# k-dominik/cluster_tools

Hardware: AMD Instinct MI355X
Metric: Gvoxel/s DT-watershed (node, 1/2/4/8 GPU) + % HBM roofline; VI vs ref (higher is better)
Workload: dtype f32

## Files before the change

### cluster_tools_amd/csrc/ctws_api.cpp

```cpp
#include <hip/hip_runtime.h>

#include <algorithm>
#include <chrono>
#include <type_traits>
#include <cmath>
#include <cstdint>
#include <cstdlib>
#include <cstdio>
#include <climits>
#include <cstring>
#include <memory>
#include <string>
#include <thread>
#include <utility>
#include <vector>

#include "../../include/ctws.h"
#include "ctws_kernels.h"
#include "host_pool.h"

using namespace ctws;

namespace {

// ... 11 lines not shown
    uint64_t* W = nullptr;
    uint32_t *Wp = nullptr, *csum = nullptr;
    uint32_t *smin = nullptr, *smax = nullptr, *sb = nullptr, *slmax = nullptr, *soff = nullptr, *surv = nullptr;
    uint32_t *act0 = nullptr, *act1 = nullptr, *lines0 = nullptr, *lines1 = nullptr;
    BlockDesc* desc = nullptr;
    BlockStat* stat = nullptr;
    uint32_t* counter = nullptr;
    double* taps = nullptr;
    int64_t cap_hash = 0;
    uint64_t* hkey = nullptr;
    uint32_t* hpos = nullptr;
    uint32_t* p2err = nullptr;
    int64_t cap_front = 0;
    uint64_t *front0 = nullptr, *front1 = nullptr, *fopen = nullptr;
    uint64_t* fplat = nullptr;
    uint64_t* fseed = nullptr;
    uint32_t* plev = nullptr;
    uint32_t* fflags = nullptr;
    uint32_t *fchunk0 = nullptr, *fchunk1 = nullptr;
    uint32_t *wl0 = nullptr, *wl1 = nullptr, *qgen = nullptr;
    uint32_t* wlcnt = nullptr;
    int64_t cap_fstat = 0;
    uint32_t* fstat = nullptr;
};

constexpr int kCounterBytes = 4 * (4 + 4 * kStatSlots);
constexpr int kFrontierBatch = 8;
constexpr int kFrontierWavesHost = 4;
constexpr int kFrontierMaxIters = 256;
constexpr int kFrontierMaxItersCap = 4096;

}

struct ctws_handle {
    int device = 0;
    hipStream_t stream = nullptr;
    std::string err;
    Workspace ws;
    uint32_t* h_counter = nullptr;
    double* h_taps = nullptr;
    std::vector<std::pair<const char*, float>> timings;
    std::vector<hipEvent_t> events;
    hipEvent_t fev[2] = {nullptr, nullptr};
    uint64_t flood_tiles = 0, flood_iters = 0, flood_lines = 0;
    DevBuf st_in, st_mask, st_init, st_out;
    struct HostSlot {
// ... 17 lines not shown
    DevBuf fs_vals, fs_sorted, fs_off, fs_tmp;
    DevBuf sf_ids, sf_bits, sf_desc, sf_stat, sf_seeds, sf_lab, sf_hm, sf_out;
    DevBuf rg_lab, rg_tab, rg_nodes, rg_pairs, rg_w, rg_keys, rg_skeys, rg_sw, rg_sum, rg_out, rg_tmp, rg_red;
    DevBuf ef_lab, ef_data, ef_nodes, ef_edges, ef_out, ef_ekeys, ef_keys, ef_skeys, ef_tmp, ef_red;
    DevBuf ov_lab, ov_rows;
    DevBuf mo_rows, mo_acc;
    DevBuf rf_data, rf_rows, rf_cnt, rf_off, rf_sums, rf_ctab;
    DevBuf ds_in, ds_out, ds_flag;
    std::vector<uint32_t> ds_flags;
    int64_t sf_n = 0;
    uint64_t sf_lo = 1, sf_hi = 0;
    bool sf_has_bits = false;
    DevBuf tc_P, tc_bits, tc_cnt, tc_offs, tc_woff, tc_red, tc_in, tc_mask, tc_out, tc_raw, tc_tmp, tc_taps;
    DevBuf ev_ka, ev_ca, ev_kb, ev_cb, ev_kp, ev_cp, ev_state, ev_out, ev_stage;
    int64_t ev_cap_a = 0, ev_cap_b = 0, ev_cap_p = 0;
    int stop_after = 0;
    int trace = 0;
    int no_descent = 0;
    int seed_tilecc = 0;
    int no_fallback = 0;
    int force_wide = 0;
    int wide_rerun = 0;
    int sf_sparse = 1;
    int verify = 1;
    int prep_lds = 0;
    int plateau_fill = 1;
    int output_tile = 1;
    int gauss_w = 0;
    int gauss_yx = 1;
    int words_per_wave = 32;
    int d2h_wgs = 0;
    int pack_threads = 6;
    int unpack_threads = 9;
    std::unique_ptr<ctws_host::WorkerPool> pack_pool, unpack_pool;
    int h2d_mode = 0;
    int h2d_wgs = 64;
    int host_ramp = 1;
    int host_batch_blocks = 0;
    int64_t host_batch_voxels = (int64_t)256 << 20;
    int edt_wz = 0;
    int edt_bits = 1;
    int edt_w = 0;
    int fchunk2[3] = {1, 64, 1};
    int fchunk3[3] = {1, 8, 8};
    int fchunk3_masked[3] = {1, 8, 8};
    int fchunk3_env = 0;
// ... 114 lines not shown
        ALLOC(hkey, hash);
        ALLOC(hpos, hash);
        w.cap_hash = hash;
    }
    if (!w.p2err) ALLOC(p2err, 4);
    if (front > w.cap_front) {
        ALLOC(front0, front);
        ALLOC(front1, front);
        ALLOC(fopen, front);
        ALLOC(fplat, front);
        ALLOC(fseed, front);
        ALLOC(fchunk0, (front >> kChunkShift) + 1);
        ALLOC(fchunk1, (front >> kChunkShift) + 1);
        ALLOC(wl0, (front >> kChunkShift) + 1);
        ALLOC(wl1, (front >> kChunkShift) + 1);
        ALLOC(qgen, (front >> kChunkShift) + 1);
        w.cap_front = front;
    }
    if (!w.fflags) ALLOC(fflags, kFrontierBatch);
    if (!w.wlcnt) ALLOC(wlcnt, kFrontierMaxItersCap + 2);
    if (blocks > w.cap_fstat) {
        ALLOC(fstat, 3 * blocks);
        ALLOC(plev, blocks);
        w.cap_fstat = blocks;
    }
    if (!w.counter) ALLOC(counter, kCounterBytes / 4);
    if (!w.taps) ALLOC(taps, 6 * kTapSlot);
#undef ALLOC
    return CTWS_OK;
}

std::vector<double> gaussian_taps(double sigma) {
    std::vector<double> k;
    if (sigma > 0.0) {
        const double sigma2 = -0.5 / sigma / sigma;
        const double norm = 1.0 / (std::sqrt(2.0 * M_PI) * sigma);
        int radius = (int)(3.0 * sigma + 0.5);
        if (radius == 0) radius = 1;
        for (double x = -(double)radius; x <= (double)radius; ++x) {
            const double x2 = x * x;
            k.push_back(norm * std::exp(x2 * sigma2));
        }
    } else {
        k.push_back(1.0);
    }
    double sum = 0.0;
// ... 983 lines not shown
        else
            k_fs_label<uint32_t><<<vg, 256, 0, h->stream>>>(w.desc, w.stat, w.hkey, w.hpos, w.hm, w.lab, w.key, w.cls,
                                                            packed ? 1 : 0);
        k_fs_auto_label<<<vg, 256, 0, h->stream>>>(w.desc, w.stat, w.surv, w.W, w.Wp, w.hm, w.lab, w.key, w.cls,
                                                   packed ? 1 : 0);
    } else {
        if (!cc_seeds)
            k_seed_label<<<rg, 256, 0, h->stream>>>(w.desc, w.stat, w.PF, w.fseed, w.hm, w.lab, w.key, w.cls,
                                                    packed ? 1 : 0);
        k_slice_seed_base<<<gsb, 256, 0, h->stream>>>(w.desc, w.stat, w.W, w.Wp, w.sb);
    }
    LAUNCHCHK();
    mark("seeds");
    if (h->stop_after == CTWS_STOP_SEEDS) {
        HIPCHK(hipStreamSynchronize(h->stream));
        return CTWS_OK;
    }

    int rounds1 = 0, rounds2 = 0;
    h->flood_tiles = h->flood_iters = h->flood_lines = 0;
    float fk1 = 0.f, fk2 = 0.f;
    int fallback = 0, fiters = 0, fiters2 = 0;
    uint32_t* fst = h->trace ? w.fstat : nullptr;
    if (descent) {
        const int dz = pl.nd_ws == 3 ? 16 : 1, dy = pl.nd_ws == 3 ? 16 : 64, dx = pl.nd_ws == 3 ? 16 : 64;
        const dim3 dg(tiles8(((maxZ + dz - 1) / dz) * ((maxY + dy - 1) / dy) * ((maxX + dx - 1) / dx)), nb);
        {
            if (pl.nd_ws == 3) k_descent_tile<3><<<dg, 512, 0, h->stream>>>(w.desc, w.stat, w.hm, w.lab, cc, w.fseed, w.P);
            else k_descent_tile<2><<<dg, 512, 0, h->stream>>>(w.desc, w.stat, w.hm, w.lab, cc, w.fseed, w.P);
            LAUNCHCHK();
        }
        mark("descent_tile");
        if (fst) HIPCHK(hipMemsetAsync(fst, 0, sizeof(uint32_t) * 2 * (size_t)nb, h->stream));
        bool any_mask = false;
        for (int i = 0; i < nb; ++i) any_mask |= desc[i].mask != nullptr;
        const bool plat_fill = h->plateau_fill && packed && any_mask;
        if (plat_fill) HIPCHK(hipMemsetAsync(w.plev, 0, sizeof(uint32_t) * (size_t)nb, h->stream));
        k_descent_init<8><<<wtg, 256, 0, h->stream>>>(w.desc, w.stat, w.hm, w.P, w.key, w.cls, w.fopen,
                                                     w.front0, fst, plat_fill ? w.plev : nullptr);
        LAUNCHCHK();
        if (plat_fill) {
            HIPCHK(hipMemsetAsync(w.fplat, 0, sizeof(uint64_t) * (size_t)TF, h->stream));
            k_plat_mark<<<wtg, 256, 0, h->stream>>>(w.desc, w.stat, w.hm, w.plev, w.fopen, w.fplat);
            LAUNCHCHK();
        }
        mark("flood_descent");
// ... 8 lines not shown
            k_plat_scan_col<1><<<dim3(cols_g, nb), 256, 0, h->stream>>>(w.desc, w.stat, w.key, w.fplat, w.plev);
            if (pl.nd_ws == 3)
                k_plat_scan_col<2><<<dim3(cols_g, nb), 256, 0, h->stream>>>(w.desc, w.stat, w.key, w.fplat, w.plev);
            k_plat_restore<<<dim3((unsigned)std::min<int64_t>(((int64_t)maxZ * maxY * ((maxX + 63) / 64) + 255) / 256, 4096), nb), 256, 0, h->stream>>>(w.desc, w.stat, w.fopen, w.fplat,
                                                                                  w.front0);
            LAUNCHCHK();
            if ((r = run_frontier(h, pl, nb, TF, max_tiles, TT, packed, fst, &fiters, &rounds1, &fk1)) != CTWS_OK)
                return r;
        }
        mark("flood_relax");
        if (fst) {
            std::vector<uint32_t> hs(2 * (size_t)nb);
            HIPCHK(hipMemcpyAsync(hs.data(), fst, sizeof(uint32_t) * 2 * (size_t)nb, hipMemcpyDeviceToHost, h->stream));
            HIPCHK(hipStreamSynchronize(h->stream));
            double no = 0, nv = 0;
            for (int i = 0; i < nb; ++i) {
                no += hs[i];
                nv += hs[nb + i];
            }
            add_timing(h, "open_voxels", (float)no);
            add_timing(h, "frontier_visits", (float)nv);
        }
        HIPCHK(hipMemsetAsync(w.counter, 0, 40, h->stream));
        if (pl.nd_ws == 3)
            k_flood_verify<3><<<wtg, 256, 0, h->stream>>>(w.desc, w.stat, w.hm, w.key, w.fopen, w.counter);
        else
            k_flood_verify<2><<<wtg, 256, 0, h->stream>>>(w.desc, w.stat, w.hm, w.key, w.fopen, w.counter);
        LAUNCHCHK();
        if (h->verify) {
            HIPCHK(hipMemcpyAsync(h->h_counter, w.counter, 40, hipMemcpyDeviceToHost, h->stream));
            HIPCHK(hipStreamSynchronize(h->stream));
            if (h->trace && h->h_counter[0]) {
                fprintf(stderr, "[ctws] flood verify: violations at");
                for (uint32_t k = 0; k < std::min(8u, h->h_counter[1]); ++k) fprintf(stderr, " %u", h->h_counter[2 + k]);
                fprintf(stderr, "\n");
            }
            if (h->h_counter[0] && h->verify >= 2) {
                h->err = "flood fixpoint check failed (CTWS_VERIFY=2)";
                return CTWS_EHIP;
            }
            if (h->h_counter[0] && !h->no_fallback) {
                fallback = 1;
                k_flood_reset<<<vg, 256, 0, h->stream>>>(w.desc, w.stat, w.hm, w.lab, cc, w.fseed, w.key, w.cls);
                LAUNCHCHK();
                if ((r = run_flood(h, pl.nd_ws, packed, nb, max_tiles, TT, w.hm, false, &rounds1, &fk1)) != CTWS_OK)
                    return r;
            }
        }
        mark("flood_verify");
    } else {
        mark("flood_descent");
        if ((r = run_flood(h, pl.nd_ws, packed, nb, max_tiles, TT, w.hm, false, &rounds1, &fk1)) != CTWS_OK) return r;
    }
    bool rerun_done = false;
    auto stop_dsat = [&]() -> int {
        if (!packed) return CTWS_OK;
        std::vector<BlockStat> sd(nb);
        HIPCHK(hipMemcpyAsync(sd.data(), w.stat, sizeof(BlockStat) * nb, hipMemcpyDeviceToHost, h->stream));
        HIPCHK(hipStreamSynchronize(h->stream));
        bool any = false;
        for (auto& x : sd) any |= x.active && x.dsat;
        if (!any) return CTWS_OK;
        ++h->wide_rerun;
        const int rr = run_batch(h, cfg, pl, blocks, io, nb);
        --h->wide_rerun;
        rerun_done = true;
        return rr;
    };
    if (h->stop_after == CTWS_STOP_FLOOD) {
        if ((r = stop_dsat()) != CTWS_OK || rerun_done) return r;
    }
    if (packed && h->stop_after == CTWS_STOP_FLOOD)
        k_unpack_labels<<<vg, 256, 0, h->stream>>>(w.desc, w.stat, w.key, w.lab);
    mark("flood");
    if (h->stop_after == CTWS_STOP_FLOOD) {
        HIPCHK(hipStreamSynchronize(h->stream));
        return CTWS_OK;
    }

    std::vector<uint32_t> surv(TS, 1u);
    int n_auto_blocks = 0;
    int n_sf_sparse = 0, n_sf_redo = 0;
    bool regrow_bad = false;
    if (cfg->size_filter > 0) {
        uint32_t* counts = (uint32_t*)w.A;
        auto histogram = [&]() -> int {
            k_hist_zero<<<vg, 256, 0, h->stream>>>(w.desc, w.stat, counts);
            if (pl.nd_ws == 2) {
                const dim3 g2((unsigned)maxZ * 4, nb);
                if (packed) k_hist2d<1><<<g2, 256, 0, h->stream>>>(w.desc, w.stat, w.lab, w.key, w.sb, counts, 4);
                else k_hist2d<0><<<g2, 256, 0, h->stream>>>(w.desc, w.stat, w.lab, w.key, w.sb, counts, 4);
            } else {
                dim3 hg((unsigned)std::min<int64_t>((maxN + 32767) / 32768, 2048), nb);
                const int bins = (int64_t)max_seeds + 1 <= kHistBins ? (int)max_seeds + 1 : 0;
                const size_t lds = sizeof(uint32_t) * (size_t)bins;
                if (packed) k_hist<1><<<hg, 256, lds, h->stream>>>(w.desc, w.stat, w.lab, w.key, counts, bins);
                else k_hist<0><<<hg, 256, lds, h->stream>>>(w.desc, w.stat, w.lab, w.key, counts, bins);
            }
            LAUNCHCHK();
            return CTWS_OK;
        };
        if ((r = histogram()) != CTWS_OK) return r;
        if (packed) {
            std::vector<BlockStat> s3(nb);
            const bool sparse_ok = h->sf_sparse && !pl.from_seeds && cfg->size_filter <= 64;
            const uint32_t* rootpos = pl.pass2 ? (const uint32_t*)w.dt : (const uint32_t*)w.Bf;
            auto regrow_init = [&]() -> int {
                HIPCHK(hipMemsetAsync(w.surv, 0, sizeof(uint32_t) * TS, h->stream));
                if (sparse_ok) {
                    k_sf_plan<<<nb, 256, 0, h->stream>>>(w.desc, w.stat, (uint32_t)cfg->size_filter, counts, excl,
                                                         w.sb, w.surv);
                    HIPCHK(hipMemsetAsync(w.fopen, 0, sizeof(uint64_t) * (size_t)TF, h->stream));
                    HIPCHK(hipMemsetAsync(w.front0, 0, sizeof(uint64_t) * (size_t)TF, h->stream));
                    k_sf_sparse<<<dim3((unsigned)std::max<uint32_t>((max_seeds + 255) / 256, 1u), nb), 256, 0,
                                   h->stream>>>(w.desc, w.stat, (uint32_t)cfg->size_filter, counts, excl,
                                                rootpos, w.hm, w.key, w.cls, w.fopen, w.front0);
                    LAUNCHCHK();
                }
                k_regrow_init<4><<<wtg, 256, 0, h->stream>>>(w.desc, w.stat, (uint32_t)cfg->size_filter, counts,
                                                            excl, w.hm, w.key, w.cls, w.fopen, w.front0, w.surv);
                LAUNCHCHK();
                HIPCHK(hipMemcpyAsync(surv.data(), w.surv, sizeof(uint32_t) * TS, hipMemcpyDeviceToHost, h->stream));
                HIPCHK(hipMemcpyAsync(s3.data(), w.stat, sizeof(BlockStat) * nb, hipMemcpyDeviceToHost, h->stream));
                HIPCHK(hipStreamSynchronize(h->stream));
                return CTWS_OK;
            };
            if ((r = regrow_init()) != CTWS_OK) return r;
            for (int i = 0; i < nb; ++i) {
                if (!s3[i].active) continue;
                const int ns = pl.nd_ws == 2 ? desc[i].Z : 1;
                bool need = false;
                for (int z = 0; z < ns; ++z) need |= !surv[desc[i].sbase + z];
                n_auto_blocks += need;
                n_sf_sparse += sparse_ok && s3[i].sf_sparse;
// ... 168 lines not shown
        sbh.resize(TS);
        inmask.resize(TS);
        HIPCHK(hipMemcpyAsync(sbh.data(), w.sb, sizeof(uint32_t) * TS, hipMemcpyDeviceToHost, h->stream));
        HIPCHK(hipMemcpyAsync(inmask.data(), w.smin, sizeof(uint32_t) * TS, hipMemcpyDeviceToHost, h->stream));
        if (pl.nd_ws == 2) {
            soffh.resize(TS);
            HIPCHK(hipMemcpyAsync(soffh.data(), w.soff, sizeof(uint32_t) * TS, hipMemcpyDeviceToHost, h->stream));
        }
    }
    HIPCHK(hipStreamSynchronize(h->stream));
    for (size_t i = 1; i < ev; ++i) {
        float ms = 0.f;
        hipEventElapsedTime(&ms, h->events[i - 1], h->events[i]);
        add_timing(h, names[i], ms);
    }
    add_timing(h, "flood_rounds", (float)rounds1);
    add_timing(h, "frontier_iters", (float)fiters);
    add_timing(h, "regrow_iters", (float)fiters2);
    add_timing(h, "flood_fallback", (float)fallback);
    add_timing(h, "regrow_rounds", (float)rounds2);
    add_timing(h, "auto_seeded_blocks", (float)n_auto_blocks);
    add_timing(h, "sf_sparse_blocks", (float)n_sf_sparse);
    add_timing(h, "sf_redo_blocks", (float)n_sf_redo);
    add_timing(h, "flood_kernel_ms", fk1);
    add_timing(h, "flood_packed", packed ? 1.f : 0.f);
    add_timing(h, "flood_tiles_solved", (float)h->flood_tiles);
    add_timing(h, "flood_local_iters", (float)h->flood_iters);
    add_timing(h, "flood_lines_swept", (float)h->flood_lines);
    add_timing(h, "size_filter_kernel_ms", fk2);
    std::vector<int> wide;
    if (packed)
        for (int i = 0; i < nb; ++i)
            if (st[i].active && st[i].dsat) wide.push_back(i);
    auto in_wide = [&](int i) { return std::find(wide.begin(), wide.end(), i) != wide.end(); };
    std::vector<int> redo;
    std::vector<std::vector<uint32_t>> redo_hint;
    if (pl.pass2 && pl.nd_ws == 2) {
        for (int i = 0; i < nb; ++i) {
            if (!st[i].active || in_wide(i)) continue;
            std::vector<uint32_t> so(soffh.begin() + desc[i].sbase, soffh.begin() + desc[i].sbase + desc[i].Z);
            const bool again = desc[i].p2hint < 0 ? (st[i].err & kErrCollision) != 0 : so != h->p2_hints[i];
            if (!again || (st[i].err & ~kErrCollision)) continue;
            if (h->p2_depth > desc[i].Z + 1) continue;
            redo.push_back(i);
            redo_hint.push_back(std::move(so));
        }
// ... 524 lines not shown
    return CTWS_OK;
}

}

extern "C" {

int ctws_abi_version(void) { return CTWS_ABI_VERSION; }

int ctws_open(int device, ctws_handle** out) {
    if (!out) return CTWS_EINVAL;
    *out = nullptr;
    int n = 0;
    if (hipGetDeviceCount(&n) != hipSuccess || n <= 0) return CTWS_EHIP;
    if (device < 0 || device >= n) return CTWS_EINVAL;
    ctws_handle* h = new ctws_handle();
    h->device = device;
    if (const char* t = std::getenv("CTWS_TRACE")) h->trace = std::atoi(t);
    if (const char* t = std::getenv("CTWS_NO_DESCENT")) h->no_descent = std::atoi(t);
    if (const char* t = std::getenv("CTWS_SEED_TILECC")) h->seed_tilecc = std::atoi(t);
    if (const char* t = std::getenv("CTWS_NO_FALLBACK")) h->no_fallback = std::atoi(t);
    if (const char* t = std::getenv("CTWS_FORCE_WIDE")) h->force_wide = std::atoi(t);
    if (const char* t = std::getenv("CTWS_SF_SPARSE")) h->sf_sparse = std::atoi(t);
    if (const char* t = std::getenv("CTWS_VERIFY")) h->verify = std::atoi(t);
    if (const char* t = std::getenv("CTWS_PREP_LDS")) h->prep_lds = std::atoi(t);
    if (const char* t = std::getenv("CTWS_EDT_BITS")) h->edt_bits = std::atoi(t);
    if (const char* t = std::getenv("CTWS_FRONTIER_ITERS"))
        h->frontier_max_iters = std::max(0, std::min(kFrontierMaxItersCap, std::atoi(t)));
    if (const char* t = std::getenv("CTWS_GAUSS_YX")) h->gauss_yx = std::atoi(t);
    if (const char* t = std::getenv("CTWS_HOST_BATCH_VOXELS")) h->host_batch_voxels = std::max<int64_t>(1, std::atoll(t));
    if (const char* t = std::getenv("CTWS_HOST_RAMP")) h->host_ramp = std::atoi(t);
    if (const char* t = std::getenv("CTWS_PLATEAU_FILL")) h->plateau_fill = std::atoi(t);
    if (const char* t = std::getenv("CTWS_OUTPUT_TILE")) h->output_tile = std::atoi(t);
    if (const char* t = std::getenv("CTWS_H2D_MODE")) h->h2d_mode = std::atoi(t);
    if (const char* t = std::getenv("CTWS_H2D_WGS")) h->h2d_wgs = std::max(1, std::atoi(t));
    if (const char* t = std::getenv("CTWS_HOST_BATCH_BLOCKS")) h->host_batch_blocks = std::max(0, std::atoi(t));
    if (const char* t = std::getenv("CTWS_PACK_THREADS")) h->pack_threads = std::max(1, std::atoi(t));
    if (const char* t = std::getenv("CTWS_UNPACK_THREADS")) h->unpack_threads = std::max(1, std::atoi(t));
    if (const char* t = std::getenv("CTWS_D2H_WGS")) h->d2h_wgs = std::max(0, std::atoi(t));
    if (const char* t = std::getenv("CTWS_WORDS_PER_WAVE")) h->words_per_wave = std::max(1, std::atoi(t));
    if (const char* t = std::getenv("CTWS_GAUSS_W")) {
        const int v = std::atoi(t);
        h->gauss_w = (v == 8 || v == 16 || v == 32) ? v : 0;
    }
    if (const char* t = std::getenv("CTWS_EDT_W")) {
        const int v = std::atoi(t);
// ... 17 lines not shown
        h->fchunk3_env = 1;
    }
    if (const char* t = std::getenv("CTWS_FRONTIER_GRID")) h->frontier_grid = std::max(1, std::atoi(t));
    if (const char* t = std::getenv("CTWS_FRONTIER_REPS")) h->frontier_reps = std::max(1, std::atoi(t));
    if (const char* t = std::getenv("CTWS_FRONTIER_DIR")) h->frontier_dir = std::atoi(t) ? 1 : 0;
    if (hipSetDevice(device) != hipSuccess || hipStreamCreateWithFlags(&h->stream, hipStreamNonBlocking) != hipSuccess ||
        hipHostMalloc((void**)&h->h_counter, kCounterBytes, hipHostMallocDefault) != hipSuccess ||
        hipHostMalloc((void**)&h->h_taps, 6 * kTapSlot * sizeof(double), hipHostMallocDefault) != hipSuccess) {
        delete h;
        return CTWS_EHIP;
    }
    *out = h;
    return CTWS_OK;
}

void ctws_close(ctws_handle* h) {
    if (!h) return;
    hipSetDevice(h->device);
    hipStreamSynchronize(h->stream);
    Workspace& w = h->ws;
    void* ptrs[] = {w.fin, w.dt, w.A, w.Bf, w.sm, w.hm, w.cls, w.P, w.PF, w.lab, w.key, w.W, w.Wp, w.csum,
                    w.smin, w.smax, w.sb, w.slmax, w.soff, w.surv, w.act0, w.act1, w.lines0, w.lines1, w.desc, w.stat, w.counter,
                    w.taps, w.hkey, w.hpos, w.p2err, w.front0, w.front1, w.fopen, w.fflags, w.fchunk0, w.fchunk1, w.wl0, w.wl1, w.qgen, w.wlcnt,
                    w.fstat, h->st_in.p, h->st_mask.p, h->st_init.p, h->st_out.p, h->rl_lab.p, h->rl_bits.p,
                    h->rl_cnt.p, h->rl_offs.p, h->rl_out.p, h->rl_keys.p, h->rl_vals.p, h->rl_red.p,
                    h->edt_fh.p, h->edt_scratch.p, h->p2_hint_dev.p, h->rl_sorted.p, h->rl_uniq.p, h->rl_counts.p, h->rl_tmp.p,
                    h->fs_vals.p, h->fs_sorted.p, h->fs_off.p, h->fs_tmp.p, h->sf_ids.p, h->sf_bits.p, h->sf_desc.p,
                    h->sf_stat.p, h->sf_seeds.p, h->sf_lab.p, h->sf_hm.p, h->sf_out.p, h->ev_ka.p, h->ev_ca.p, h->ev_kb.p,
                    h->ev_cb.p, h->ev_kp.p, h->ev_cp.p, h->ev_state.p, h->ev_out.p, h->ev_stage.p,
                    w.fplat, w.plev, w.fseed, h->tc_P.p, h->tc_bits.p, h->tc_cnt.p, h->tc_offs.p, h->tc_woff.p,
                    h->tc_red.p, h->tc_in.p, h->tc_mask.p, h->tc_out.p, h->tc_raw.p, h->tc_tmp.p, h->tc_taps.p,
                    h->rg_lab.p, h->rg_tab.p, h->rg_nodes.p, h->rg_pairs.p, h->rg_w.p, h->rg_keys.p, h->rg_skeys.p, h->rg_sw.p,
                    h->rg_sum.p, h->rg_out.p, h->rg_tmp.p, h->rg_red.p, h->ef_lab.p, h->ef_data.p, h->ef_nodes.p,
                    h->ef_edges.p, h->ef_out.p, h->ef_ekeys.p, h->ef_keys.p, h->ef_skeys.p, h->ef_tmp.p, h->ef_red.p,
                    h->ov_lab.p, h->ov_rows.p, h->mo_rows.p, h->mo_acc.p, h->rf_data.p, h->rf_rows.p,
                    h->rf_cnt.p, h->rf_off.p, h->rf_sums.p, h->rf_ctab.p, h->ds_in.p, h->ds_out.p,
                    h->ds_flag.p};
    for (void* p : ptrs)
        if (p) hipFree(p);
    for (auto e : h->events) hipEventDestroy(e);
    for (auto e : h->fev)
        if (e) hipEventDestroy(e);
    if (h->h_counter) hipHostFree(h->h_counter);
    if (h->h_taps) hipHostFree(h->h_taps);
    for (auto& sl : h->hslot) {
        if (sl.pin_in) hipHostFree(sl.pin_in);
        if (sl.pin_out) hipHostFree(sl.pin_out);
// ... 1783 lines not shown
```

### cluster_tools_amd/csrc/ctws_dev.h

```cpp
#pragma once

#include <hip/hip_runtime.h>
#include <stdint.h>

namespace ctws {

constexpr uint32_t kInfD2 = 0x3FFFFFFFu;
constexpr uint64_t kInfKey = 0xFFFFFFFFFFFFFFFFull;
constexpr uint32_t kNoParent = 0xFFFFFFFFu;
constexpr uint32_t kFixedBit = 0x80000000u;
constexpr uint32_t kRootBit = 0x80000000u;
constexpr int kRows = 4;
constexpr uint32_t kDescRes = 0x80000000u;

struct BlockDesc {
    int Z, Y, X, nd_ws;
    int64_t N;
    int64_t base;
    int iz0, iy0, ix0, crop;
    int IZ, IY, IX, _p0;
    int64_t NI;
    int64_t ibase;
    int64_t wbase;
    int64_t cbase;
// ... 305 lines not shown
            (void)z;                                                                                         \
            (void)y;                                                                                         \
            __VA_ARGS__                                                                                      \
        }                                                                                                    \
    }

__device__ __forceinline__ int div_small(int n, int d, float inv) {
    int q = (int)((float)n * inv);
    const int r = n - q * d;
    q += r < 0 ? -1 : (r >= d ? 1 : 0);
    return q;
}

__device__ __forceinline__ uint64_t shfl_up_u64(uint64_t v, int d) {
    return (uint64_t)__shfl_up((long long)v, d);
}
__device__ __forceinline__ uint64_t shfl_u64(uint64_t v, int src) {
    return (uint64_t)__shfl((long long)v, src);
}
__device__ __forceinline__ uint64_t shfl_down_u64(uint64_t v, int d) {
    return (uint64_t)__shfl_down((long long)v, d);
}

constexpr uint64_t kPackInf = ~0ull;
constexpr uint32_t kLabelBits = 20;
constexpr uint64_t kLabelMask = (1ull << kLabelBits) - 1ull;
constexpr uint64_t kDOne = 1ull << kLabelBits;
constexpr uint64_t kDMask = 0xFFFull << kLabelBits;
constexpr uint32_t kDMax = 4095;

__device__ __forceinline__ bool key_dsat(uint64_t k) { return (k & kDMask) == kDMask && k != kPackInf; }
__device__ __forceinline__ void note_dsat(const BlockStat* S, int b) {
    uint32_t* p = const_cast<uint32_t*>(&S[b].dsat);
    if (!*(volatile uint32_t*)p) atomicOr(p, 1u);
}

__device__ __forceinline__ uint64_t f_packed(uint32_t hb, uint64_t best) {
    const uint32_t c = (uint32_t)(best >> 32);
    if (hb > c) return ((uint64_t)hb << 32) | (best & kLabelMask);
    return ((best & kDMask) >= ((uint64_t)kDMax << kLabelBits)) ? best : best + kDOne;
}

__device__ __forceinline__ bool is_seed(const uint32_t* lab, const uint32_t* cc, int64_t gi) {
    return cc ? cc[gi] != kNoParent : (lab[gi] & kFixedBit) != 0;
}

// ... 8 lines not shown
```

### cluster_tools_amd/csrc/ctws_kernels.h

```cpp
#pragma once

#include "ctws_dev.h"

namespace ctws {

struct PrepParams {
    float threshold;
    int invert;
    int agg;
    int px2;
};
struct EdtColParams {
    int axis;
    int p2;
    int final_pass;
    int per_slice;
    uint32_t max_dist;
    int px2;
};
struct EdtRealParams {
    double pitch[3];
    int per_slice;
    int real;
};
// ... 171 lines not shown
                             const int* beg, const int* end, hipStream_t stream);
hipError_t fs_segmented_sort(void* tmp, size_t& bytes, const uint64_t* in, uint64_t* out, int n, int nseg,
                             const int* beg, const int* end, hipStream_t stream);
struct SfDiscard {
    const uint64_t* ids;
    int64_t n;
    const uint64_t* bits;
    uint64_t lo, hi;
};
struct SfBlock {
    const uint64_t* lab;
    uint64_t* seeds;
    int64_t N;
};
__global__ void k_sf_member(const SfBlock*, BlockStat*, SfDiscard);
__global__ void k_sf_hmap(const BlockDesc*, float*);
constexpr int kChunkShift = 6;
template <int CW, int CY, int CZ>
__global__ void k_frontier_list0(const BlockDesc*, const BlockStat*, const uint64_t*, uint32_t*, uint32_t*);
__global__ void k_frontier_tiles(const BlockDesc*, const BlockStat*, const uint64_t*, uint32_t*, int, int, int);
template <int ND>
__global__ void k_flood_verify(const BlockDesc*, const BlockStat*, const float*, const uint64_t*, const uint64_t*,
                               uint32_t*);
constexpr int kWordWaves = 4;
__global__ void k_flood_reset(const BlockDesc*, const BlockStat*, const float*, const uint32_t*, const uint32_t*,
                              const uint64_t*, uint64_t*, uint8_t*);

__global__ void k_slice_seed_base(const BlockDesc*, const BlockStat*, const uint64_t*, const uint32_t*, uint32_t*);
__global__ void k_hist_zero(const BlockDesc*, const BlockStat*, uint32_t*);
template <int PACKED>
__global__ void k_hist(const BlockDesc*, const BlockStat*, const uint32_t*, const uint64_t*, uint32_t*, int);
constexpr int kHistBins = 16384;
__global__ void k_size_filter(const BlockDesc*, const BlockStat*, FilterParams, const uint32_t*, const uint8_t*,
                              const float*, uint32_t*, uint64_t*, uint8_t*, uint32_t*, int);
__global__ void k_slice_max(const BlockDesc*, const BlockStat*, const uint32_t*, const uint64_t*, int, const uint32_t*,
                            uint32_t*, int, int);
template <int PACKED>
__global__ void k_hist2d(const BlockDesc*, const BlockStat*, const uint32_t*, const uint64_t*, const uint32_t*,
                         uint32_t*, int);
__global__ void k_sf_plan(const BlockDesc*, BlockStat*, uint32_t, const uint32_t*, const uint8_t*, const uint32_t*,
                          uint32_t*);
__global__ void k_sf_sparse(const BlockDesc*, BlockStat*, uint32_t, const uint32_t*, const uint8_t*,
                            const uint32_t*, const float*, uint64_t*, uint8_t*, uint64_t*, uint64_t*);
__global__ void k_fixed_from_open(const BlockDesc*, const BlockStat*, const uint64_t*, uint8_t*);
template <int U>
__global__ void k_regrow_init(const BlockDesc*, const BlockStat*, uint32_t, const uint32_t*, const uint8_t*,
                              const float*, uint64_t*, uint8_t*, uint64_t*, uint64_t*, uint32_t*);
__global__ void k_auto_minima(const BlockDesc*, const BlockStat*, const float*, const uint32_t*, uint64_t*);
__global__ void k_auto_seed_set(const BlockDesc*, BlockStat*, const float*, const uint32_t*, const uint64_t*,
                                const uint32_t*, const uint32_t*, uint64_t*, uint8_t*, uint64_t*, uint64_t*, uint32_t*);
__global__ void k_slice_offsets(const BlockDesc*, const BlockStat*, const uint32_t*, uint32_t*);
__global__ void k_finalize_ws(const BlockDesc*, const BlockStat*, const uint32_t*, const uint32_t*, const uint64_t*, int,
                              uint32_t*);

__global__ void k_p2_zero_dt(const BlockDesc*, const BlockStat*, float*);
__global__ void k_p2_insert(const BlockDesc*, BlockStat*, uint64_t*, uint32_t*, const uint32_t*, const uint64_t*,
                            const uint32_t*, const uint32_t*);
__global__ void k_p2_roots(const BlockDesc*, const BlockStat*, const uint64_t*, const uint32_t*, uint64_t*);
__global__ void k_p2_label(const BlockDesc*, const BlockStat*, const uint64_t*, const uint32_t*, const uint64_t*,
                           const uint32_t*, const float*, uint32_t*, uint64_t*, uint8_t*, uint32_t*, uint32_t*, int, int,
                           const uint32_t*, const uint64_t*, const uint32_t*, const uint32_t*, uint8_t*);
__global__ void k_p2_excl_zero(const BlockDesc*, const BlockStat*, uint8_t*);
__global__ void k_p2_excl(const BlockDesc*, const BlockStat*, const uint32_t*, uint8_t*);
__global__ void k_p2_check(const BlockDesc*, BlockStat*, const uint64_t*, const uint32_t*);
// ... 146 lines not shown
```

### cluster_tools_amd/csrc/k_flood.hip

```cpp
#include <type_traits>

#include "ctws_kernels.h"

namespace ctws {

template <int ND>
struct FloodTile;
template <>
struct FloodTile<3> {
    static constexpr int TZ = 4, TY = 8, TX = 64, HZ = TZ + 2;
};
template <>
struct FloodTile<2> {
    static constexpr int TZ = 1, TY = 32, TX = 64, HZ = 1;
};

__device__ __forceinline__ void take_min(uint64_t nk, uint32_t nl, uint64_t& bk, uint32_t& bl) {
    if (nk < bk || (nk == bk && nl < bl)) {
        bk = nk;
        bl = nl;
    }
}

__device__ __forceinline__ uint64_t f_key(uint32_t hb, uint64_t bk) {
// ... 1154 lines not shown
            if (ND == 3) {
                if (z > 0) m = min(m, kzm[u]);
                if (z + 1 < B.Z) m = min(m, kzp[u]);
            }
            const uint64_t e = (m == kPackInf) ? kPackInf : f_packed(ordf(hv[u]), m);
            const bool b1 = valid && ((ow[u] >> lane) & 1ull) && e != o;
            dsat |= valid && ((ow[u] >> lane) & 1ull) && key_dsat(o);
            if (b1 && flag[1] < 8u) {
                const uint32_t slot = atomicAdd(&flag[1], 1u);
                if (slot < 8u) flag[2 + slot] = (uint32_t)(B.base + zb + (int64_t)y * B.X + x);
            }
            bad |= b1;
        }
      }
    }
    if (__ballot(bad) && (threadIdx.x & 63) == 0) atomicOr(flag, 1u);
    if (__ballot(dsat) && (threadIdx.x & 63) == 0) note_dsat(S, blockIdx.y);
}
template __global__ void k_flood_verify<3>(const BlockDesc*, const BlockStat*, const float*, const uint64_t*,
                                           const uint64_t*, uint32_t*);
template __global__ void k_flood_verify<2>(const BlockDesc*, const BlockStat*, const float*, const uint64_t*,
                                           const uint64_t*, uint32_t*);

__global__ void __launch_bounds__(256) k_flood_reset(const BlockDesc* __restrict__ D, const BlockStat* S,
                                                     const float* __restrict__ h, const uint32_t* __restrict__ lab,
                                                     const uint32_t* __restrict__ cc, const uint64_t* __restrict__ sbits,
                                                     uint64_t* __restrict__ key, uint8_t* __restrict__ fixedv) {
    const BlockDesc& B = D[blockIdx.y];
    if (!S[blockIdx.y].active) return;
    for (int64_t i = (int64_t)blockIdx.x * blockDim.x + threadIdx.x; i < B.N; i += (int64_t)gridDim.x * blockDim.x) {
        const uint32_t l = (!cc || bit_of(sbits, B, i)) ? seed_label(lab, cc, B.base, (uint32_t)i) : 0u;
        key[B.base + i] = l ? (((uint64_t)ordf(h[B.base + i]) << 32) | (uint64_t)l) : kPackInf;
        fixedv[B.base + i] = l ? 1 : 0;
    }
}

}
```

### cluster_tools_amd/csrc/k_post.hip

```cpp
#include "ctws_kernels.h"

namespace ctws {

#define BLOCK_LOOP(i, B)                                                                      \
    for (int64_t i = (int64_t)blockIdx.x * blockDim.x + threadIdx.x; i < (B).N;              \
         i += (int64_t)gridDim.x * blockDim.x)

__global__ void __launch_bounds__(256) k_slice_seed_base(const BlockDesc* __restrict__ D, const BlockStat* S,
                                                         const uint64_t* __restrict__ W,
                                                         const uint32_t* __restrict__ Wp, uint32_t* sb) {
    const BlockDesc& B = D[blockIdx.y];
    if (!S[blockIdx.y].active) return;
    const int z = blockIdx.x * blockDim.x + threadIdx.x;
    if (z >= B.Z) return;
    const uint32_t f = (uint32_t)((int64_t)z * B.Y * B.X);
    sb[B.sbase + z] = (B.nd_ws == 2) ? bitmap_rank(W + B.wbase, Wp + B.wbase, f) : 0u;
}

__global__ void __launch_bounds__(256) k_hist_zero(const BlockDesc* __restrict__ D, const BlockStat* S,
                                                   uint32_t* __restrict__ counts) {
    const BlockDesc& B = D[blockIdx.y];
    if (!S[blockIdx.y].active) return;
    const int64_t n = (int64_t)S[blockIdx.y].n_seeds + 1;
    for (int64_t i = (int64_t)blockIdx.x * blockDim.x + threadIdx.x; i < n; i += (int64_t)gridDim.x * blockDim.x)
        counts[B.base + i] = 0;
}

template <class Add>
__device__ __forceinline__ void count_label_runs(uint32_t l, bool ok, int lane, Add add) {
    const uint32_t prev = (uint32_t)__shfl_up((int)l, 1);
    const uint64_t act = __ballot(ok);
    const uint64_t starts = __ballot(ok && (lane == 0 || prev != l));
    if (!((starts >> lane) & 1ull)) return;
    const uint64_t ends = (starts | ~act) & ~((2ull << lane) - 1ull);
    const int next = ends ? __builtin_ctzll(ends) : 64;
    add(l, (uint32_t)(next - lane));
}

template <int PACKED>
__global__ void __launch_bounds__(256) k_hist(const BlockDesc* __restrict__ D, const BlockStat* S,
                                              const uint32_t* __restrict__ lab, const uint64_t* __restrict__ key,
                                              uint32_t* __restrict__ counts, int bins) {
    extern __shared__ uint32_t sh[];
    const BlockDesc& B = D[blockIdx.y];
    if (!S[blockIdx.y].active) return;
    uint32_t* c = counts + B.base;
    const int64_t nb = (int64_t)S[blockIdx.y].n_seeds + 1;
    const bool use_lds = nb <= bins;
    if (use_lds)
        for (int j = threadIdx.x; j < nb; j += 256) sh[j] = 0;
    __syncthreads();
    const int64_t chunk = ((B.N + gridDim.x - 1) / gridDim.x + 255) & ~(int64_t)255;
    const int64_t i0 = (int64_t)blockIdx.x * chunk, i1 = min(B.N, i0 + chunk);
    const int lane = threadIdx.x & 63;
    constexpr int U = 8;
    for (int64_t ib = i0; ib < i1; ib += 256 * U) {
        uint32_t lv[U];
#pragma unroll
        for (int u = 0; u < U; ++u) {
// ... 6 lines not shown
                lv[u] = lab[ic] & ~kFixedBit;
            }
        }
#pragma unroll
        for (int u = 0; u < U; ++u) {
            const int64_t i = ib + u * 256 + threadIdx.x;
            lv[u] = i >= i1 ? 0xFFFFFFFFu : ((lv[u] & 0x80000000u) ? 0u : lv[u]);
        }
#pragma unroll
        for (int u = 0; u < U; ++u) {
            const uint32_t l = lv[u];
            count_label_runs(l, l != 0xFFFFFFFFu, lane, [&](uint32_t lb, uint32_t n) {
                if (use_lds) atomicAdd(&sh[lb], n);
                else atomicAdd(&c[lb], n);
            });
        }
    }
    if (!use_lds) return;
    __syncthreads();
    for (int j = threadIdx.x; j < nb; j += 256)
        if (sh[j]) atomicAdd(&c[j], sh[j]);
}

constexpr int kHist2dBins = 8192;
template <int PACKED>
__global__ void __launch_bounds__(256) k_hist2d(const BlockDesc* __restrict__ D, const BlockStat* S,
                                                const uint32_t* __restrict__ lab, const uint64_t* __restrict__ key,
                                                const uint32_t* __restrict__ sb, uint32_t* __restrict__ counts,
                                                int splits) {
    __shared__ uint32_t sh[kHist2dBins];
    const BlockDesc& B = D[blockIdx.y];
    if (!S[blockIdx.y].active) return;
    const int z = blockIdx.x / splits, s = blockIdx.x % splits;
    if (z >= B.Z) return;
    const uint32_t b0 = sb[B.sbase + z];
    const uint32_t b1 = z + 1 < B.Z ? sb[B.sbase + z + 1] : S[blockIdx.y].n_seeds;
    const uint32_t nb = b1 - b0;
    const bool use_lds = nb <= (uint32_t)kHist2dBins;
    if (use_lds)
        for (uint32_t j = threadIdx.x; j < nb; j += 256) sh[j] = 0;
    __syncthreads();
    const int64_t YX = (int64_t)B.Y * B.X;
    const int64_t i0 = (int64_t)z * YX + YX * s / splits, i1 = (int64_t)z * YX + YX * (s + 1) / splits;
    uint32_t* c = counts + B.base + b0 + 1;
    const int lane = threadIdx.x & 63;
    constexpr int U = 8;
    for (int64_t ib = i0; ib < i1; ib += 256 * U) {
// ... 18 lines not shown
        for (int u = 0; u < U; ++u) {
            const uint32_t l = lv[u];
            count_label_runs(l, l != 0xFFFFFFFFu, lane, [&](uint32_t lb, uint32_t n) {
                if (lb <= b0 || lb > b1) return;
                if (use_lds) atomicAdd(&sh[lb - b0 - 1], n);
                else atomicAdd(&c[lb - b0 - 1], n);
            });
        }
    }
    if (!use_lds) return;
    __syncthreads();
    for (uint32_t j = threadIdx.x; j < nb; j += 256)
        if (sh[j]) atomicAdd(&c[j], sh[j]);
}

constexpr uint32_t kSfSparseMax = 64;

__device__ __forceinline__ bool sf_keeps(const uint32_t* c, const uint8_t* ex, uint32_t l, uint32_t size_filter) {
    return c[l] >= size_filter || (ex && ex[l]);
}

__global__ void __launch_bounds__(256) k_sf_plan(const BlockDesc* __restrict__ D, BlockStat* S, uint32_t size_filter,
                                                 const uint32_t* __restrict__ counts, const uint8_t* __restrict__ excl,
                                                 const uint32_t* __restrict__ sb, uint32_t* __restrict__ survivors) {
    const BlockDesc& B = D[blockIdx.x];
    BlockStat& st = S[blockIdx.x];
    if (!st.active) return;
    const uint32_t ns = st.n_seeds;
    const uint32_t* c = counts + B.base;
    const uint8_t* ex = excl ? excl + B.base : nullptr;
    uint32_t nsmall = 0, tot = 0;
    for (uint32_t l = 1 + threadIdx.x; l <= ns; l += 256) {
        nsmall += sf_keeps(c, ex, l, size_filter) ? 0u : 1u;
        tot += c[l];
    }
    nsmall = wg_reduce_u32(nsmall, OpAdd());
    tot = wg_reduce_u32(tot, OpAdd());
    uint32_t bare = 0;
    if (B.nd_ws == 2) {
        for (int z = threadIdx.x; z < B.Z; z += 256) {
            const uint32_t l0 = sb[B.sbase + z], l1 = z + 1 < B.Z ? sb[B.sbase + z + 1] : ns;
            bool any = false;
            for (uint32_t l = l0 + 1; l <= l1 && !any; ++l) any = sf_keeps(c, ex, l, size_filter);
            bare += any ? 0u : 1u;
        }
    } else {
        bare = threadIdx.x == 0 && nsmall == ns ? 1u : 0u;
    }
    bare = wg_reduce_u32(bare, OpAdd());
    const uint32_t unreached = (uint32_t)B.N - tot;
    const bool sparse = size_filter <= kSfSparseMax && !unreached && !bare &&
                        (uint64_t)nsmall * size_filter <= (uint64_t)B.N / 8;
    if (threadIdx.x == 0) {
        st.sf_sparse = sparse ? 1u : 0u;
        st.sf_redo = 0u;
    }
    if (sparse)
        for (int z = threadIdx.x; z < (B.nd_ws == 2 ? B.Z : 1); z += 256) survivors[B.sbase + z] = 1u;
}

__global__ void __launch_bounds__(256) k_sf_sparse(const BlockDesc* __restrict__ D, BlockStat* S,
                                                   uint32_t size_filter, const uint32_t* __restrict__ counts,
                                                   const uint8_t* __restrict__ excl,
                                                   const uint32_t* __restrict__ rootpos, const float* __restrict__ h,
                                                   uint64_t* __restrict__ key, uint8_t* __restrict__ fixedv,
                                                   uint64_t* __restrict__ open, uint64_t* __restrict__ chg) {
    const BlockDesc& B = D[blockIdx.y];
    BlockStat& st = S[blockIdx.y];
    if (!st.active || !st.sf_sparse) return;
    const uint32_t l = 1u + blockIdx.x * blockDim.x + threadIdx.x;
    if (l > st.n_seeds) return;
    const uint32_t* c = counts + B.base;
// ... 381 lines not shown
```

Before: 17.21.

## Fuse size-filter histogram into flood verify and split sf_plan across workgroups

For 2D watershed with a size filter, the flood-verify pass now also counts per-slice label runs into LDS bins. This removes the separate histogram pass that re-read the key array. The sf_plan kernel is also split across several workgroups per block, with atomic accumulators and a last-block finalisation, and its bare-slice check is vectorised with wave ballots. The costs are a more complex verify kernel, an extra label read on closed tiles, and a count recompute if fallback triggers.

```diff
diff --git a/cluster_tools_amd/csrc/ctws_api.cpp b/cluster_tools_amd/csrc/ctws_api.cpp
--- a/cluster_tools_amd/csrc/ctws_api.cpp
+++ b/cluster_tools_amd/csrc/ctws_api.cpp
@@ -57,6 +57,7 @@
     uint32_t* wlcnt = nullptr;
     int64_t cap_fstat = 0;
     uint32_t* fstat = nullptr;
+    uint32_t* sfacc = nullptr;
 };
 
 constexpr int kCounterBytes = 4 * (4 + 4 * kStatSlots);
@@ -120,6 +121,7 @@
     int force_wide = 0;
     int wide_rerun = 0;
     int sf_sparse = 1;
+    int fuse_hist = 1;
     int verify = 1;
     int prep_lds = 0;
     int plateau_fill = 1;
@@ -280,6 +282,8 @@
     if (blocks > w.cap_fstat) {
         ALLOC(fstat, 3 * blocks);
         ALLOC(plev, blocks);
+        ALLOC(sfacc, 4 * blocks);
+        HIPCHK(hipMemsetAsync(w.sfacc, 0, sizeof(uint32_t) * 4 * (size_t)blocks, h->stream));
         w.cap_fstat = blocks;
     }
     if (!w.counter) ALLOC(counter, kCounterBytes / 4);
@@ -1309,6 +1313,10 @@
     float fk1 = 0.f, fk2 = 0.f;
     int fallback = 0, fiters = 0, fiters2 = 0;
     uint32_t* fst = h->trace ? w.fstat : nullptr;
+    uint32_t* const counts = (uint32_t*)w.A;
+    const bool fuse_hist = h->fuse_hist && descent && pl.nd_ws == 2 && !pl.pass2 && !pl.from_seeds &&
+                           cfg->size_filter > 0 && h->stop_after != CTWS_STOP_FLOOD;
+    bool counts_ready = false;
     if (descent) {
         const int dz = pl.nd_ws == 3 ? 16 : 1, dy = pl.nd_ws == 3 ? 16 : 64, dx = pl.nd_ws == 3 ? 16 : 64;
         const dim3 dg(tiles8(((maxZ + dz - 1) / dz) * ((maxY + dy - 1) / dy) * ((maxX + dx - 1) / dx)), nb);
@@ -1363,7 +1371,17 @@
             add_timing(h, "frontier_visits", (float)nv);
         }
         HIPCHK(hipMemsetAsync(w.counter, 0, 40, h->stream));
-        if (pl.nd_ws == 3)
+        if (fuse_hist) {
+            k_hist_zero<<<vg, 256, 0, h->stream>>>(w.desc, w.stat, counts);
+            int64_t per_slice = 0;
+            for (int i = 0; i < nb; ++i)
+                if (s2[i].active) per_slice = std::max<int64_t>(per_slice, (int64_t)s2[i].n_seeds / std::max(desc[i].Z, 1) + 1);
+            int bins = 512;
+            while (bins < kHist2dBins && bins < per_slice + per_slice / 2) bins *= 2;
+            k_flood_verify_hist2d<<<dim3((unsigned)maxZ * 4, nb), kVerifyHistThreads, sizeof(uint32_t) * (size_t)bins,
+                                    h->stream>>>(w.desc, w.stat, w.hm, w.key, w.fopen, w.sb, counts, w.counter, 4, bins);
+            counts_ready = true;
+        } else if (pl.nd_ws == 3)
             k_flood_verify<3><<<wtg, 256, 0, h->stream>>>(w.desc, w.stat, w.hm, w.key, w.fopen, w.counter);
         else
             k_flood_verify<2><<<wtg, 256, 0, h->stream>>>(w.desc, w.stat, w.hm, w.key, w.fopen, w.counter);
@@ -1382,6 +1400,7 @@
             }
             if (h->h_counter[0] && !h->no_fallback) {
                 fallback = 1;
+                counts_ready = false;
                 k_flood_reset<<<vg, 256, 0, h->stream>>>(w.desc, w.stat, w.hm, w.lab, cc, w.fseed, w.key, w.cls);
                 LAUNCHCHK();
                 if ((r = run_flood(h, pl.nd_ws, packed, nb, max_tiles, TT, w.hm, false, &rounds1, &fk1)) != CTWS_OK)
@@ -1424,7 +1443,6 @@
     int n_sf_sparse = 0, n_sf_redo = 0;
     bool regrow_bad = false;
     if (cfg->size_filter > 0) {
-        uint32_t* counts = (uint32_t*)w.A;
         auto histogram = [&]() -> int {
             k_hist_zero<<<vg, 256, 0, h->stream>>>(w.desc, w.stat, counts);
             if (pl.nd_ws == 2) {
@@ -1441,7 +1459,7 @@
             LAUNCHCHK();
             return CTWS_OK;
         };
-        if ((r = histogram()) != CTWS_OK) return r;
+        if (!counts_ready && (r = histogram()) != CTWS_OK) return r;
         if (packed) {
             std::vector<BlockStat> s3(nb);
             const bool sparse_ok = h->sf_sparse && !pl.from_seeds && cfg->size_filter <= 64;
@@ -1449,8 +1467,9 @@
             auto regrow_init = [&]() -> int {
                 HIPCHK(hipMemsetAsync(w.surv, 0, sizeof(uint32_t) * TS, h->stream));
                 if (sparse_ok) {
-                    k_sf_plan<<<nb, 256, 0, h->stream>>>(w.desc, w.stat, (uint32_t)cfg->size_filter, counts, excl,
-                                                         w.sb, w.surv);
+                    const unsigned split = std::min<unsigned>(kSfPlanSplit, max_seeds / kSfPlanLabels + 1);
+                    k_sf_plan<<<dim3(split, nb), 256, 0, h->stream>>>(
+                        w.desc, w.stat, (uint32_t)cfg->size_filter, counts, excl, w.sb, w.surv, w.sfacc);
                     HIPCHK(hipMemsetAsync(w.fopen, 0, sizeof(uint64_t) * (size_t)TF, h->stream));
                     HIPCHK(hipMemsetAsync(w.front0, 0, sizeof(uint64_t) * (size_t)TF, h->stream));
                     k_sf_sparse<<<dim3((unsigned)std::max<uint32_t>((max_seeds + 255) / 256, 1u), nb), 256, 0,
@@ -1665,6 +1684,7 @@
     add_timing(h, "auto_seeded_blocks", (float)n_auto_blocks);
     add_timing(h, "sf_sparse_blocks", (float)n_sf_sparse);
     add_timing(h, "sf_redo_blocks", (float)n_sf_redo);
+    add_timing(h, "hist_fused", counts_ready ? 1.f : 0.f);
     add_timing(h, "flood_kernel_ms", fk1);
     add_timing(h, "flood_packed", packed ? 1.f : 0.f);
     add_timing(h, "flood_tiles_solved", (float)h->flood_tiles);
@@ -2235,6 +2255,7 @@
     if (const char* t = std::getenv("CTWS_NO_FALLBACK")) h->no_fallback = std::atoi(t);
     if (const char* t = std::getenv("CTWS_FORCE_WIDE")) h->force_wide = std::atoi(t);
     if (const char* t = std::getenv("CTWS_SF_SPARSE")) h->sf_sparse = std::atoi(t);
+    if (const char* t = std::getenv("CTWS_FUSE_HIST")) h->fuse_hist = std::atoi(t);
     if (const char* t = std::getenv("CTWS_VERIFY")) h->verify = std::atoi(t);
     if (const char* t = std::getenv("CTWS_PREP_LDS")) h->prep_lds = std::atoi(t);
     if (const char* t = std::getenv("CTWS_EDT_BITS")) h->edt_bits = std::atoi(t);
@@ -2298,7 +2319,7 @@
     void* ptrs[] = {w.fin, w.dt, w.A, w.Bf, w.sm, w.hm, w.cls, w.P, w.PF, w.lab, w.key, w.W, w.Wp, w.csum,
                     w.smin, w.smax, w.sb, w.slmax, w.soff, w.surv, w.act0, w.act1, w.lines0, w.lines1, w.desc, w.stat, w.counter,
                     w.taps, w.hkey, w.hpos, w.p2err, w.front0, w.front1, w.fopen, w.fflags, w.fchunk0, w.fchunk1, w.wl0, w.wl1, w.qgen, w.wlcnt,
-                    w.fstat, h->st_in.p, h->st_mask.p, h->st_init.p, h->st_out.p, h->rl_lab.p, h->rl_bits.p,
+                    w.fstat, w.sfacc, h->st_in.p, h->st_mask.p, h->st_init.p, h->st_out.p, h->rl_lab.p, h->rl_bits.p,
                     h->rl_cnt.p, h->rl_offs.p, h->rl_out.p, h->rl_keys.p, h->rl_vals.p, h->rl_red.p,
                     h->edt_fh.p, h->edt_scratch.p, h->p2_hint_dev.p, h->rl_sorted.p, h->rl_uniq.p, h->rl_counts.p, h->rl_tmp.p,
                     h->fs_vals.p, h->fs_sorted.p, h->fs_off.p, h->fs_tmp.p, h->sf_ids.p, h->sf_bits.p, h->sf_desc.p,
diff --git a/cluster_tools_amd/csrc/ctws_dev.h b/cluster_tools_amd/csrc/ctws_dev.h
--- a/cluster_tools_amd/csrc/ctws_dev.h
+++ b/cluster_tools_amd/csrc/ctws_dev.h
@@ -351,6 +351,17 @@
     return (uint64_t)__shfl_down((long long)v, d);
 }
 
+template <class Add>
+__device__ __forceinline__ void count_label_runs(uint32_t l, bool ok, int lane, Add add) {
+    const uint32_t prev = (uint32_t)__shfl_up((int)l, 1);
+    const uint64_t act = __ballot(ok);
+    const uint64_t starts = __ballot(ok && (lane == 0 || prev != l));
+    if (!((starts >> lane) & 1ull)) return;
+    const uint64_t ends = (starts | ~act) & ~((2ull << lane) - 1ull);
+    const int next = ends ? __builtin_ctzll(ends) : 64;
+    add(l, (uint32_t)(next - lane));
+}
+
 constexpr uint64_t kPackInf = ~0ull;
 constexpr uint32_t kLabelBits = 20;
 constexpr uint64_t kLabelMask = (1ull << kLabelBits) - 1ull;
diff --git a/cluster_tools_amd/csrc/ctws_kernels.h b/cluster_tools_amd/csrc/ctws_kernels.h
--- a/cluster_tools_amd/csrc/ctws_kernels.h
+++ b/cluster_tools_amd/csrc/ctws_kernels.h
@@ -217,6 +217,10 @@
 template <int ND>
 __global__ void k_flood_verify(const BlockDesc*, const BlockStat*, const float*, const uint64_t*, const uint64_t*,
                                uint32_t*);
+constexpr int kHist2dBins = 8192;
+constexpr int kVerifyHistThreads = 256;
+__global__ void k_flood_verify_hist2d(const BlockDesc*, const BlockStat*, const float*, const uint64_t*,
+                                      const uint64_t*, const uint32_t*, uint32_t*, uint32_t*, int, int);
 constexpr int kWordWaves = 4;
 __global__ void k_flood_reset(const BlockDesc*, const BlockStat*, const float*, const uint32_t*, const uint32_t*,
                               const uint64_t*, uint64_t*, uint8_t*);
@@ -233,8 +237,10 @@
 template <int PACKED>
 __global__ void k_hist2d(const BlockDesc*, const BlockStat*, const uint32_t*, const uint64_t*, const uint32_t*,
                          uint32_t*, int);
+constexpr int kSfPlanSplit = 32;
+constexpr int kSfPlanLabels = 4096;
 __global__ void k_sf_plan(const BlockDesc*, BlockStat*, uint32_t, const uint32_t*, const uint8_t*, const uint32_t*,
-                          uint32_t*);
+                          uint32_t*, uint32_t*);
 __global__ void k_sf_sparse(const BlockDesc*, BlockStat*, uint32_t, const uint32_t*, const uint8_t*,
                             const uint32_t*, const float*, uint64_t*, uint8_t*, uint64_t*, uint64_t*);
 __global__ void k_fixed_from_open(const BlockDesc*, const BlockStat*, const uint64_t*, uint8_t*);
diff --git a/cluster_tools_amd/csrc/k_flood.hip b/cluster_tools_amd/csrc/k_flood.hip
--- a/cluster_tools_amd/csrc/k_flood.hip
+++ b/cluster_tools_amd/csrc/k_flood.hip
@@ -1200,6 +1200,125 @@
 template __global__ void k_flood_verify<2>(const BlockDesc*, const BlockStat*, const float*, const uint64_t*,
                                            const uint64_t*, uint32_t*);
 
+__global__ void __launch_bounds__(kVerifyHistThreads) __attribute__((amdgpu_waves_per_eu(6, 8)))
+k_flood_verify_hist2d(const BlockDesc* __restrict__ D, const BlockStat* S, const float* __restrict__ h,
+                      const uint64_t* __restrict__ key, const uint64_t* __restrict__ open,
+                      const uint32_t* __restrict__ sb, uint32_t* __restrict__ counts, uint32_t* __restrict__ flag,
+                      int splits, int bins) {
+    extern __shared__ uint32_t sh[];
+    const BlockDesc& B = D[blockIdx.y];
+    if (!S[blockIdx.y].active) return;
+    const int z = blockIdx.x / splits, s = blockIdx.x % splits;
+    if (z >= B.Z) return;
+    const uint32_t b0 = sb[B.sbase + z];
+    const uint32_t b1 = z + 1 < B.Z ? sb[B.sbase + z + 1] : S[blockIdx.y].n_seeds;
+    const uint32_t nb = b1 - b0;
+    const bool use_lds = nb <= (uint32_t)bins;
+    if (use_lds)
+        for (uint32_t j = threadIdx.x; j < nb; j += blockDim.x) sh[j] = 0;
+    __syncthreads();
+    uint32_t* c = counts + B.base + b0 + 1;
+    constexpr int U = 4, R = U + 2;
+    const int64_t zb = (int64_t)z * B.Y * B.X;
+    const int wpr = (B.X + 63) >> 6;
+    const gptr_t<uint64_t> k = gbl(key + B.base + zb);
+    const gptr_t<float> hb = gbl(h + B.base + zb);
+    const gptr_t<uint64_t> ob = gbl(open + B.fbase + (int64_t)z * B.Y * wpr);
+    const int ngy = (B.Y + U - 1) / U;
+    const int nu = wpr * ngy;
+    const int q0 = (int)((int64_t)nu * s / splits), q1 = (int)((int64_t)nu * (s + 1) / splits);
+    const int lane = threadIdx.x & 63;
+    const int nw = (int)(blockDim.x >> 6);
+    const int per = (q1 - q0 + nw - 1) / nw;
+    const int ubeg = q0 + (int)(threadIdx.x >> 6) * per, uend = min(q1, ubeg + per);
+    bool bad = false, dsat = false;
+    for (int un0 = ubeg; un0 < uend; un0 += 64) {
+        uint64_t lw[U];
+        {
+            const int ul = un0 + lane;
+            const int xwl = ul / ngy, gyl = ul - xwl * ngy;
+#pragma unroll
+            for (int u = 0; u < U; ++u)
+                lw[u] = (ul < uend && gyl * U + u < B.Y)
+                            ? ob[(gyl * U + u) * wpr + xwl]
+                            : 0ull;
+        }
+        const uint64_t has_open = __ballot((lw[0] | lw[1] | lw[2] | lw[3]) != 0ull);
+        const int cnt = min(64, uend - un0);
+        for (int src = 0; src < cnt; ++src) {
+            const int un = un0 + src;
+            const int xw = un / ngy, gy = un - xw * ngy;
+            const int y0 = gy * U;
+            const bool any_open = (has_open >> src) & 1ull;
+            const int x = xw * 64 + lane;
+            const int xc = min(x, B.X - 1);
+            const int xe = lane == 0 ? max(xc - 1, 0) : min(xc + 1, B.X - 1);
+            uint64_t rk[R];
+#pragma unroll
+            for (int q = 0; q < R; ++q) {
+                const int yy = min(max(y0 - 1 + q, 0), B.Y - 1);
+                rk[q] = k[yy * B.X + xc];
+            }
+            uint64_t ke[U];
+            float hv[U];
+            if (any_open) {
+#pragma unroll
+                for (int u = 0; u < U; ++u) {
+                    const int yy = min(y0 + u, B.Y - 1);
+                    ke[u] = k[yy * B.X + xe];
+                    hv[u] = hb[yy * B.X + xc];
+                }
+            } else {
+#pragma unroll
+                for (int u = 0; u < U; ++u) {
+                    ke[u] = kPackInf;
+                    hv[u] = 0.f;
+                }
+            }
+#pragma unroll
+            for (int u = 0; u < U; ++u) {
+                const uint64_t kv = rk[u + 1];
+                const uint32_t l = kv == kPackInf ? 0u : (uint32_t)(kv & kLabelMask);
+                count_label_runs(l, y0 + u < B.Y && x < B.X, lane, [&](uint32_t lb, uint32_t n) {
+                    if (lb <= b0 || lb > b1) return;
+                    if (use_lds) atomicAdd(&sh[lb - b0 - 1], n);
+                    else atomicAdd(&c[lb - b0 - 1], n);
+                });
+            }
+            if (!any_open) continue;
+#pragma unroll
+            for (int u = 0; u < U; ++u) {
+                const int y = y0 + u;
+                const bool valid = y < B.Y && x < B.X;
+                const uint64_t o = valid ? rk[u + 1] : kPackInf;
+                uint64_t l = shfl_up_u64(o, 1), r = shfl_down_u64(o, 1);
+                const uint64_t ker = shfl_u64(ke[u], 63);
+                if (lane == 0) l = (x > 0) ? ke[u] : kPackInf;
+                if (lane == 63) r = ker;
+                if (x + 1 >= B.X) r = kPackInf;
+                uint64_t m = min(l, r);
+                if (y > 0) m = min(m, rk[u]);
+                if (y + 1 < B.Y) m = min(m, rk[u + 2]);
+                const uint64_t e = (m == kPackInf) ? kPackInf : f_packed(ordf(hv[u]), m);
+                const bool isopen = valid && ((shfl_u64(lw[u], src) >> lane) & 1ull);
+                const bool b1v = isopen && e != o;
+                dsat |= isopen && key_dsat(o);
+                if (b1v && flag[1] < 8u) {
+                    const uint32_t slot = atomicAdd(&flag[1], 1u);
+                    if (slot < 8u) flag[2 + slot] = (uint32_t)(B.base + (int64_t)z * B.Y * B.X + y * B.X + x);
+                }
+                bad |= b1v;
+            }
+        }
+    }
+    if (__ballot(bad) && lane == 0) atomicOr(flag, 1u);
+    if (__ballot(dsat) && lane == 0) note_dsat(S, blockIdx.y);
+    if (!use_lds) return;
+    __syncthreads();
+    for (uint32_t j = threadIdx.x; j < nb; j += blockDim.x)
+        if (sh[j]) atomicAdd(&c[j], sh[j]);
+}
+
 __global__ void __launch_bounds__(256) k_flood_reset(const BlockDesc* __restrict__ D, const BlockStat* S,
                                                      const float* __restrict__ h, const uint32_t* __restrict__ lab,
                                                      const uint32_t* __restrict__ cc, const uint64_t* __restrict__ sbits,
diff --git a/cluster_tools_amd/csrc/k_post.hip b/cluster_tools_amd/csrc/k_post.hip
--- a/cluster_tools_amd/csrc/k_post.hip
+++ b/cluster_tools_amd/csrc/k_post.hip
@@ -24,17 +24,6 @@
     const int64_t n = (int64_t)S[blockIdx.y].n_seeds + 1;
     for (int64_t i = (int64_t)blockIdx.x * blockDim.x + threadIdx.x; i < n; i += (int64_t)gridDim.x * blockDim.x)
         counts[B.base + i] = 0;
-}
-
-template <class Add>
-__device__ __forceinline__ void count_label_runs(uint32_t l, bool ok, int lane, Add add) {
-    const uint32_t prev = (uint32_t)__shfl_up((int)l, 1);
-    const uint64_t act = __ballot(ok);
-    const uint64_t starts = __ballot(ok && (lane == 0 || prev != l));
-    if (!((starts >> lane) & 1ull)) return;
-    const uint64_t ends = (starts | ~act) & ~((2ull << lane) - 1ull);
-    const int next = ends ? __builtin_ctzll(ends) : 64;
-    add(l, (uint32_t)(next - lane));
 }
 
 template <int PACKED>
@@ -87,7 +76,6 @@
         if (sh[j]) atomicAdd(&c[j], sh[j]);
 }
 
-constexpr int kHist2dBins = 8192;
 template <int PACKED>
 __global__ void __launch_bounds__(256) k_hist2d(const BlockDesc* __restrict__ D, const BlockStat* S,
                                                 const uint32_t* __restrict__ lab, const uint64_t* __restrict__ key,
@@ -152,15 +140,19 @@
 
 __global__ void __launch_bounds__(256) k_sf_plan(const BlockDesc* __restrict__ D, BlockStat* S, uint32_t size_filter,
                                                  const uint32_t* __restrict__ counts, const uint8_t* __restrict__ excl,
-                                                 const uint32_t* __restrict__ sb, uint32_t* __restrict__ survivors) {
-    const BlockDesc& B = D[blockIdx.x];
-    BlockStat& st = S[blockIdx.x];
+                                                 const uint32_t* __restrict__ sb, uint32_t* __restrict__ survivors,
+                                                 uint32_t* __restrict__ acc) {
+    const BlockDesc& B = D[blockIdx.y];
+    BlockStat& st = S[blockIdx.y];
     if (!st.active) return;
     const uint32_t ns = st.n_seeds;
     const uint32_t* c = counts + B.base;
     const uint8_t* ex = excl ? excl + B.base : nullptr;
+    uint32_t* a = acc + 4 * blockIdx.y;
+    const uint32_t per = (ns + gridDim.x - 1) / gridDim.x;
+    const uint32_t la = 1u + blockIdx.x * per, lb = min(ns, la + per - 1u);
     uint32_t nsmall = 0, tot = 0;
-    for (uint32_t l = 1 + threadIdx.x; l <= ns; l += 256) {
+    for (uint32_t l = la + threadIdx.x; l <= lb; l += 256) {
         nsmall += sf_keeps(c, ex, l, size_filter) ? 0u : 1u;
         tot += c[l];
     }
@@ -168,16 +160,34 @@
     tot = wg_reduce_u32(tot, OpAdd());
     uint32_t bare = 0;
     if (B.nd_ws == 2) {
-        for (int z = threadIdx.x; z < B.Z; z += 256) {
+        const int lane = threadIdx.x & 63;
+        for (int z = blockIdx.x * 4 + (threadIdx.x >> 6); z < B.Z; z += gridDim.x * 4) {
             const uint32_t l0 = sb[B.sbase + z], l1 = z + 1 < B.Z ? sb[B.sbase + z + 1] : ns;
             bool any = false;
-            for (uint32_t l = l0 + 1; l <= l1 && !any; ++l) any = sf_keeps(c, ex, l, size_filter);
-            bare += any ? 0u : 1u;
-        }
-    } else {
-        bare = threadIdx.x == 0 && nsmall == ns ? 1u : 0u;
+            for (uint32_t l = l0 + 1; l <= l1 && !any; l += 64)
+                any = __ballot(l + lane <= l1 && sf_keeps(c, ex, l + lane, size_filter)) != 0ull;
+            bare += (lane == 0 && !any) ? 1u : 0u;
+        }
     }
     bare = wg_reduce_u32(bare, OpAdd());
+    __shared__ uint32_t last, totals[3];
+    if (threadIdx.x == 0) {
+        atomicAdd(&a[0], nsmall);
+        atomicAdd(&a[1], tot);
+        atomicAdd(&a[2], bare);
+        __threadfence();
+        last = atomicAdd(&a[3], 1u) == gridDim.x - 1 ? 1u : 0u;
+        if (last) {
+            __threadfence();
+            for (int j = 0; j < 3; ++j) totals[j] = atomicAdd(&a[j], 0u);
+            for (int j = 0; j < 4; ++j) a[j] = 0u;
+        }
+    }
+    __syncthreads();
+    if (!last) return;
+    nsmall = totals[0];
+    tot = totals[1];
+    bare = B.nd_ws == 2 ? totals[2] : (nsmall == ns ? 1u : 0u);
     const uint32_t unreached = (uint32_t)B.N - tot;
     const bool sparse = size_filter <= kSfSparseMax && !unreached && !bare &&
                         (uint64_t)nsmall * size_filter <= (uint64_t)B.N / 8;
```

Result: faster. 17.51 (median of 6 runs) (+1.7%).
